# YongonY/NBLDPC

Measured on AMD Instinct MI355X. Metric: decoded codewords/sec @ 50 iters, GF(256) N=512 rate-1/2, higher is better.
Workload: dtype f64

## Files before the change

### nbldpc_amd/csrc/nbl_api.cpp

```cpp
#include <hip/hip_runtime.h>
#include <cstdio>
#include <cstdlib>
#include <cstring>
#include <chrono>
#include <cmath>
#include <string>
#include <thread>
#include <vector>
#include "../../include/nbldpc.h"
#include "nbl_kernels.h"
#include "nbl_osd.h"

static thread_local std::string g_create_error;

struct nbl_decoder {
	int device = -1;
	nbl_params prm{};
	nbl_params_ext ext{};
	bool osd_on = false;
	bool osd_acc = false;
	NblOsdDev osd{};
	double osd_factor = 0.0;
	double *osd_S = nullptr;
	NblGraphDev g{};
	NblWork w{};
	std::vector<void *> graph_allocs;
	int *d_e2c_map = nullptr;
	int cap = 0;
	size_t ws_bytes = 0;
	double *d_Lin = nullptr;
	uint8_t *d_conv8 = nullptr;
	hipStream_t stream = nullptr;
	bool record_state = false;
	bool all_dc4 = false;
	int min_dc = 0;
	bool all_dv2 = false;
	double *c2v_alt = nullptr;
	double *c2v_zero = nullptr;
	const double *last_c2v = nullptr;
	bool last_fused = false;
	int dm_order = 0, dm_L = 0;
	double *d_cons = nullptr;
	int *d_src = nullptr;
	double *d_rx = nullptr;
	size_t d_rx_cap = 0;
	std::vector<double> h_cons;
	uint32_t *d_jump = nullptr;
	uint32_t *d_state = nullptr;
	uint8_t *d_txi = nullptr;
	double *d_fn = nullptr;
	uint32_t *d_fidx = nullptr;
	double *d_farg = nullptr, *d_fval = nullptr;
	unsigned *d_fcount = nullptr;
	uint32_t *h_fidx = nullptr;
	double *h_farg = nullptr, *h_fval = nullptr;
	size_t noise_cap = 0, flag_cap = 0;
	double last_flag_frac = 0.0;
	hipStream_t stream2 = nullptr;
	double *d_rxs[2] = {nullptr, nullptr};
	size_t d_rxs_cap[2] = {0, 0};
	int rxs_B[2] = {0, 0};
	struct Tx {
		bool on = false;
		int crc_len = 0, random_msg = 0, K = 0, nb = 0, nw = 0, nwg = 0, mb = 0, period = 1, par_mod = 0;
		unsigned long long *T = nullptr, *G = nullptr;
		int *keep = nullptr;
		uint32_t *crc_col = nullptr;
		int16_t *phase_of = nullptr;
		uint8_t *seq = nullptr;
		uint16_t *pn = nullptr;
		unsigned long long *u = nullptr;
		uint8_t *bits = nullptr;
		size_t cap = 0;
		uint8_t *code[2] = {nullptr, nullptr}, *txi[2] = {nullptr, nullptr};
		size_t slot_cap[2] = {0, 0};
		int tx_B[2] = {0, 0};
		int *dec[2] = {nullptr, nullptr};
		size_t dec_cap[2] = {0, 0};
// ... 10 lines not shown
	int *d_active = nullptr;
	bool use_compact = true;
	bool use_graph = false;
	int force_generic = 0;
	bool profiling = false;
	hipEvent_t ev[2] = {nullptr, nullptr};
	int *h_ndone = nullptr;
	std::vector<hipEvent_t> pev;
	double ms[4] = {0, 0, 0, 0};
	long long launches[3] = {0, 0, 0};
	int last_B = 0;
	std::vector<int> h_coff, h_cvar, h_ch;
	std::vector<uint16_t> h_mul;
	std::string err;
};

#define HIP_TRY_E(errstr, call)                                                                    \
	do {                                                                                           \
		hipError_t e_ = (call);                                                                    \
		if (e_ != hipSuccess) {                                                                    \
			(errstr) = std::string(#call) + ": " + hipGetErrorString(e_);                          \
			return NBL_ERR_HIP;                                                                    \
		}                                                                                          \
	} while (0)
#define HIP_TRY(dec, call) HIP_TRY_E((dec)->err, call)

static int ilog2(int q)
{
	int p = 0;
	while ((1 << p) < q) p++;
	return p;
}

template <typename T> static nbl_status upload(nbl_decoder *d, const std::vector<T> &h, const T **dst)
{
	void *p = nullptr;
	HIP_TRY(d, hipMalloc(&p, h.size() * sizeof(T) + 16));
	d->graph_allocs.push_back(p);
	HIP_TRY(d, hipMemcpy(p, h.data(), h.size() * sizeof(T), hipMemcpyHostToDevice));
	*dst = (const T *)p;
	return NBL_OK;
}

static void drop_graphs(nbl_decoder *d)
{
	for (auto &ge : d->gexec)
		if (ge) (void)hipGraphExecDestroy(ge);
	d->gexec.clear();
}

static void free_workspace(nbl_decoder *d)
{
	drop_graphs(d);
	void *ptrs[] = {d->w.Lch, d->w.v2c, d->w.c2v, d->w.post, d->w.dec, d->w.out, d->w.iters, d->w.done, d->d_Lin, d->d_conv8, d->c2v_alt, d->w.edge_dec, d->d_active, d->c2v_zero, d->osd_S};
	d->osd_S = nullptr;
	d->c2v_zero = nullptr;
	d->d_active = nullptr;
	d->w.active = nullptr;
	d->c2v_alt = nullptr;
	for (void *p : ptrs)
		if (p) (void)hipFree(p);
	d->w.Lch = d->w.v2c = d->w.c2v = d->w.post = nullptr;
	d->w.dec = d->w.out = d->w.iters = d->w.edge_dec = nullptr;
	d->w.done = nullptr;
	d->d_Lin = nullptr;
	d->d_conv8 = nullptr;
	d->cap = 0;
	d->ws_bytes = 0;
}

static bool small_enabled()
{
	static const bool on = !getenv("NBL_NO_SMALL");
	return on;
}

static bool small_shape(const nbl_decoder *d)
{
	if (!small_enabled()) return false;
	const nbl_params &p = d->prm;
	if (p.method == NBL_METHOD_TEMS && d->all_dv2 && nbl_tems64_applicable(d->g, d->all_dc4, p.tems_nr, p.tems_nc)) return false;
	if (p.method == NBL_METHOD_BP && nbl_bp64_applicable(d->g, d->all_dc4)) return false;
	if (p.method == NBL_METHOD_EMS) return nbl_small_applicable(d->g, p.method, d->min_dc, p.ems_nm, p.ems_nc);
	if (p.method == NBL_METHOD_TEMS) return nbl_small_applicable(d->g, p.method, d->min_dc, 0, p.tems_nc);
	if (p.method == NBL_METHOD_BP) return nbl_small_applicable(d->g, p.method, d->min_dc, 0, 0);
	return false;
}

static bool ems64_shape(const nbl_decoder *d)
{
	return small_enabled() && d->prm.method == NBL_METHOD_EMS && nbl_ems64_applicable(d->g, d->min_dc, d->prm.ems_nm, d->prm.ems_nc);
}

static bool fused_shape(const nbl_decoder *d)
{
	if (small_shape(d) || ems64_shape(d)) return d->g.c_nbr != nullptr;
	if (!d->all_dv2) return false;
	if (d->prm.method == NBL_METHOD_EMS) return nbl_ems256_applicable(d->g, d->all_dc4, d->prm.ems_nm, d->prm.ems_nc);
	if (d->prm.method == NBL_METHOD_TEMS)
		return nbl_tems64_applicable(d->g, d->all_dc4, d->prm.tems_nr, d->prm.tems_nc) || nbl_tems256_applicable(d->g, d->all_dc4, d->prm.tems_nr, d->prm.tems_nc);
	if (d->prm.method == NBL_METHOD_BP) return nbl_bp256_applicable(d->g, d->all_dc4) || nbl_bp64_applicable(d->g, d->all_dc4);
	return false;
}

static nbl_status ensure_workspace(nbl_decoder *d, int B)
{
	const bool want_v2c = d->prm.method != NBL_METHOD_EMS || !fused_shape(d) || d->record_state || d->force_generic != 0;
	const bool want_post = d->record_state || d->osd_acc;
	if (B <= d->cap && (!want_post || d->w.post) && (!want_v2c || d->w.v2c)) return NBL_OK;
	int cap = B > d->cap ? B : d->cap;
	free_workspace(d);
	const size_t q = d->g.q, N = d->g.N, E = d->g.E;
	size_t bytes = 0;
	auto alloc = [&](void **p, size_t n) -> hipError_t { bytes += n; return hipMalloc(p, n); };
	HIP_TRY(d, alloc((void **)&d->w.Lch, (size_t)cap * N * q * 8));
	if (want_v2c) HIP_TRY(d, alloc((void **)&d->w.v2c, (size_t)cap * E * q * 8));
	HIP_TRY(d, alloc((void **)&d->w.c2v, (size_t)cap * E * q * 8));
	if (fused_shape(d)) {
		HIP_TRY(d, alloc((void **)&d->c2v_alt, (size_t)cap * E * q * 8));
		HIP_TRY(d, alloc((void **)&d->c2v_zero, E * q * 8));
		HIP_TRY(d, hipMemset(d->c2v_zero, 0, E * q * 8));
	}
	if (want_post) HIP_TRY(d, alloc((void **)&d->w.post, (size_t)cap * N * q * 8));
	if (d->osd_acc) HIP_TRY(d, alloc((void **)&d->osd_S, (size_t)cap * N * d->g.p * 8));
	HIP_TRY(d, alloc((void **)&d->w.dec, (size_t)cap * N * 4));
	if (d->prm.method != NBL_METHOD_EMS) HIP_TRY(d, alloc((void **)&d->w.edge_dec, (size_t)cap * E * 4));
	HIP_TRY(d, alloc((void **)&d->w.out, (size_t)cap * N * 4));
	HIP_TRY(d, alloc((void **)&d->w.iters, (size_t)cap * 4));
	HIP_TRY(d, alloc((void **)&d->w.done, (size_t)cap));
	HIP_TRY(d, alloc((void **)&d->d_active, (size_t)cap * 4));
	d->cap = cap;
	d->ws_bytes = bytes;
	return NBL_OK;
}

extern "C" int32_t nbl_abi_version(void) { return NBL_ABI_VERSION; }

extern "C" const char *nbl_last_error(const nbl_decoder *dec)
{
	if (!dec) return g_create_error.c_str();
	if (dec->err2.empty()) return dec->err.c_str();
	if (dec->err.empty()) return dec->err2.c_str();
	static thread_local std::string both;
	both = dec->err + " | channel: " + dec->err2;
	return both.c_str();
}

extern "C" size_t nbl_workspace_bytes(const nbl_decoder *dec) { return dec ? dec->ws_bytes : 0; }

static nbl_status fail_create(nbl_decoder *d, nbl_status st, const std::string &msg)
{
	g_create_error = msg.empty() && d ? d->err : msg;
	if (d) nbl_destroy(d);
	return st;
}

extern "C" nbl_status nbl_create(const nbl_code_desc *code, const uint16_t *gf_mul, const uint16_t *gf_inv,
                                 const nbl_params *params, int device, nbl_decoder **out)
{
	return nbl_create_ex(code, gf_mul, gf_inv, params, nullptr, device, out);
}

extern "C" nbl_status nbl_create_ex(const nbl_code_desc *code, const uint16_t *gf_mul, const uint16_t *gf_inv,
                                    const nbl_params *params, const nbl_params_ext *ext, int device, nbl_decoder **out)
{
	return nbl_create_osd(code, gf_mul, gf_inv, params, ext, nullptr, device, out);
}

static void g_gauss_eliminate(std::vector<std::vector<uint8_t>> &m, int col_length, int row_length, std::vector<int> &order)
{
	for (int row = 0; row < row_length; row++) {
		int col = order[row];
		if (m[row][col] == 0) {
			bool exchanged = false;
			for (int up = row + 1; up < row_length; up++)
				if (m[up][col] != 0) {
					for (int i = 0; i < col_length; i++) m[row][i] ^= m[up][i];
					exchanged = true;
					break;
				}
			if (!exchanged) {
				const int flag = row;
				row--;
// ... 280 lines not shown
	(void)hipDeviceSynchronize();
	free_workspace(d);
	for (void *p : d->graph_allocs) (void)hipFree(p);
	if (d->d_src) (void)hipFree(d->d_src);
	if (d->d_cons) (void)hipFree(d->d_cons);
	if (d->d_rx) (void)hipFree(d->d_rx);
	for (double *p : d->d_rxs)
		if (p) (void)hipFree(p);
	if (d->stream2) { (void)hipStreamSynchronize(d->stream2); (void)hipStreamDestroy(d->stream2); }
	for (void *p : {(void *)d->d_jump, (void *)d->d_state, (void *)d->d_txi, (void *)d->d_fn, (void *)d->d_fidx, (void *)d->d_farg, (void *)d->d_fval, (void *)d->d_fcount})
		if (p) (void)hipFree(p);
	for (void *p : {(void *)d->h_fidx, (void *)d->h_farg, (void *)d->h_fval})
		if (p) (void)hipHostFree(p);
	free_transmitter(d);
	for (auto &e : d->ev)
		if (e) (void)hipEventDestroy(e);
	if (d->h_ndone) (void)hipHostFree(d->h_ndone);
	for (auto &e : d->pev) (void)hipEventDestroy(e);
	if (d->stream) (void)hipStreamDestroy(d->stream);
	delete d;
}

extern "C" nbl_status nbl_set_profiling(nbl_decoder *d, int32_t on)
{
	if (!d) return NBL_ERR_ARG;
	d->profiling = on != 0;
	return NBL_OK;
}

extern "C" nbl_status nbl_debug_force_generic(nbl_decoder *d, int32_t on)
{
	if (!d) return NBL_ERR_ARG;
	d->force_generic = on;
	return NBL_OK;
}

extern "C" int32_t nbl_debug_graph_windows(nbl_decoder *d)
{
	int n = 0;
	if (d)
		for (auto &ge : d->gexec) n += ge != nullptr;
	return n;
}

extern "C" nbl_status nbl_debug_stamps(nbl_decoder *d, int32_t on, unsigned long long out[16])
{
	if (!d) return NBL_ERR_ARG;
	d->err.clear();
	HIP_TRY(d, hipSetDevice(d->device));
	if (out && d->w.stamps) {
		HIP_TRY(d, hipStreamSynchronize(d->stream));
		HIP_TRY(d, hipDeviceSynchronize());
		HIP_TRY(d, hipMemcpy(out, d->w.stamps, 16 * 8, hipMemcpyDeviceToHost));
	}
	if (on && !d->w.stamps) {
		void *p = nullptr;
		HIP_TRY(d, hipMalloc(&p, 16 * 8));
		d->graph_allocs.push_back(p);
		d->w.stamps = (unsigned long long *)p;
	}
	if (d->w.stamps && on) HIP_TRY(d, hipMemset(d->w.stamps, 0, 16 * 8));
	if (!on) d->w.stamps = nullptr;
	return NBL_OK;
}

extern "C" nbl_status nbl_set_record_state(nbl_decoder *d, int32_t on)
{
	if (!d) return NBL_ERR_ARG;
	d->record_state = on != 0;
	return NBL_OK;
}

extern "C" nbl_status nbl_last_timing(nbl_decoder *d, double ms[4], int64_t launches[3])
{
	if (!d) return NBL_ERR_ARG;
	if (ms) memcpy(ms, d->ms, sizeof d->ms);
	if (launches) for (int i = 0; i < 3; i++) launches[i] = d->launches[i];
	return NBL_OK;
}

static nbl_status launch_cn(nbl_decoder *d, const NblRun &r, hipStream_t st)
{
	const bool small_on = small_shape(d);
	switch (d->prm.method) {
	case NBL_METHOD_EMS:
		if (d->force_generic != 1 && nbl_ems256_applicable(d->g, d->all_dc4, r.nm, r.nc)) HIP_TRY(d, nbl_launch_cn_ems256(d->g, d->w, r, false, st));
		else if (d->force_generic != 1 && small_on) HIP_TRY(d, nbl_launch_cn_ems_small(d->g, d->w, r, false, st));
		else if (d->force_generic != 1 && ems64_shape(d)) HIP_TRY(d, nbl_launch_cn_ems64(d->g, d->w, r, false, st));
		else HIP_TRY(d, nbl_launch_cn_ems(d->g, d->w, r, st));
		break;
	case NBL_METHOD_TEMS:
		if (d->force_generic != 1 && nbl_tems64_applicable(d->g, d->all_dc4, r.nr, r.nc)) HIP_TRY(d, nbl_launch_cn_tems64(d->g, d->w, r, false, st));
		else if (d->force_generic != 1 && nbl_tems256_applicable(d->g, d->all_dc4, r.nr, r.nc)) HIP_TRY(d, nbl_launch_cn_tems256(d->g, d->w, r, false, st));
		else if (d->force_generic != 1 && small_on) HIP_TRY(d, nbl_launch_cn_tems_small(d->g, d->w, r, false, st));
		else HIP_TRY(d, nbl_launch_cn_tems(d->g, d->w, r, st));
		break;
	case NBL_METHOD_BP:
		if (d->force_generic != 1 && nbl_bp256_applicable(d->g, d->all_dc4)) HIP_TRY(d, nbl_launch_cn_bp256(d->g, d->w, r, false, st));
		else if (d->force_generic != 1 && nbl_bp64_applicable(d->g, d->all_dc4)) HIP_TRY(d, nbl_launch_cn_bp64(d->g, d->w, r, false, st));
		else if (d->force_generic != 1 && small_on) HIP_TRY(d, nbl_launch_cn_bp_small(d->g, d->w, r, false, st));
		else HIP_TRY(d, nbl_launch_cn_bp(d->g, d->w, r, st));
		break;
	case NBL_METHOD_BS_TEMS: HIP_TRY(d, nbl_launch_cn_bstems(d->g, d->w, r, st)); break;
	default: d->err = "check-node kernel for this method is not built yet"; return NBL_ERR_UNSUPPORTED;
	}
	return NBL_OK;
}

struct IterCtx {
	nbl_decoder *d;
	NblRun r;
	bool damp, fused;
	double *bufA, *bufB;
	const double *zeros = nullptr;
	int batch = 0;
// ... 880 lines not shown
```

### nbldpc_amd/csrc/nbl_cn_ems256.hip

```cpp
#include <hip/hip_runtime.h>
#ifndef NBL_EMS_PRUNE
#define NBL_EMS_PRUNE 1
#endif
#include <type_traits>
#include "nbl_device.h"
#include "nbl_kernels.h"

#ifndef NBL_WHATIF
#define NBL_WHATIF 0
#endif

namespace {

constexpr int Q = 256;

struct ListEnt { double v; int t8; int tt; };

#define WSYNC() __builtin_amdgcn_fence(__ATOMIC_ACQ_REL, "wavefront")

template <int CTRL, int ROW_MASK = 0xF>
__device__ __forceinline__ double dpp_mov_f64(double x)
{
	int lo = __builtin_amdgcn_update_dpp(__double2loint(x), __double2loint(x), CTRL, ROW_MASK, 0xF, false);
	int hi = __builtin_amdgcn_update_dpp(__double2hiint(x), __double2hiint(x), CTRL, ROW_MASK, 0xF, false);
	return __hiloint2double(hi, lo);
}

__device__ __forceinline__ double wave_max_f64(double x)
{
	x = dmax(x, dpp_mov_f64<0xB1>(x));
	x = dmax(x, dpp_mov_f64<0x4E>(x));
	x = dmax(x, dpp_mov_f64<0x141>(x));
	x = dmax(x, dpp_mov_f64<0x140>(x));
	x = dmax(x, dpp_mov_f64<0x142, 0xA>(x));
	x = dmax(x, dpp_mov_f64<0x143, 0xC>(x));
	return read_lane_f64(x, 63);
}

__device__ __forceinline__ int wave_scan_add(int x)
{
	x += __builtin_amdgcn_update_dpp(0, x, 0x111, 0xF, 0xF, false);
	x += __builtin_amdgcn_update_dpp(0, x, 0x112, 0xF, 0xF, false);
	x += __builtin_amdgcn_update_dpp(0, x, 0x114, 0xF, 0xF, false);
	x += __builtin_amdgcn_update_dpp(0, x, 0x118, 0xF, 0xF, false);
	x += __builtin_amdgcn_update_dpp(0, x, 0x142, 0xA, 0xF, false);
	x += __builtin_amdgcn_update_dpp(0, x, 0x143, 0xC, 0xF, false);
	return x;
}

__device__ __forceinline__ int wave_max_i32(int x)
{
	constexpr int ID = (int)0x80000000;
	auto mx = [](int a, int b) { return a > b ? a : b; };
	x = mx(x, __builtin_amdgcn_update_dpp(ID, x, 0xB1, 0xF, 0xF, false));
	x = mx(x, __builtin_amdgcn_update_dpp(ID, x, 0x4E, 0xF, 0xF, false));
// ... 122 lines not shown
		int best = -1;
#pragma unroll
		for (int i = 0; i < 4; i++) {
			const int a = __builtin_amdgcn_inverse_ballot_w64(eq[i]) ? mh.at_slot(i) : -1;
			best = a > best ? a : best;
		}
		const int amax = wave_max_i32(best);
#pragma unroll
		for (int i = 0; i < 4; i++) {
			const uint64_t hit = __ballot(__builtin_amdgcn_inverse_ballot_w64(eq[i]) && mh.at_slot(i) == amax);
			member[i] |= hit;
			eq[i] &= ~hit;
		}
	}
}

__device__ __forceinline__ void finish_members(SelState &s, int nm, uint64_t (&member)[4], int hinv, int poly, int lane)
{
	int cgt = 0, ceq = 0;
#pragma unroll
	for (int i = 0; i < 4; i++) { cgt += __popcll(s.gt[i]); ceq += __popcll(s.eq[i]); }
	const int need = nm - cgt;
#pragma unroll
	for (int i = 0; i < 4; i++) member[i] = s.gt[i];
	if (need == ceq) {
#pragma unroll
		for (int i = 0; i < 4; i++) member[i] |= s.eq[i];
	} else {
		finish_ties(member, s.eq, need, hinv, poly, lane);
	}
}

}

template <int NMT, bool FUSED, int NC>
__global__ __launch_bounds__(64) void cn_ems_q256_dc4_kernel(NblGraphDev g, NblWork w, NblRun r)
{
	constexpr int NM = NMT < 0 ? -NMT : NMT;
	constexpr bool VARNM = NMT < 0;
	const int nmr = VARNM ? r.nm : NM;
	constexpr int LOGNM = (NM == 8) ? 3 : (NM == 16) ? 4 : (NM == 32) ? 5 : 6;
#if NBL_WHATIF == 5
	__shared__ __attribute__((aligned(16))) char smem[13 * 1024];
#elif NBL_WHATIF == 6
	__shared__ __attribute__((aligned(16))) char smem[19 * 1024];
#else
	__shared__ __attribute__((aligned(16))) char smem[3 * Q * 8 + 4 * NM * 8 + 4 * NM * 8];
#endif
	const int lane = lane_id();
	const NblXcdSlot xs = nbl_xcd_slot(g.M);
	const int m = xs.unit, b = nbl_codeword(w, r, xs.slot);
	if (b < 0) return;
	if (!r.fixed_iters && w.done[b]) return;
#if NBL_EMS_PRUNE
	const bool tryf = NC >= 2 && r.fixed_iters && w.done[b];
#else
	const bool tryf = false;
#endif
	const int c0 = g.coff[m];

	double *const B0 = (double *)smem, *const B1 = B0 + Q, *const B2 = B1 + Q;
	double *const lstv = B2 + Q;
	int2 *const lstt = (int2 *)(lstv + 4 * NM);
	auto list_at = [&](int j, int k) {
		ListEnt e;
		e.v = lstv[j * NM + k];
		const int2 o = lstt[j * NM + k];
		e.t8 = o.x;
		e.tt = o.y;
		return e;
	};

#ifdef NBL_EMS_STAMPS
	unsigned long long st_t0 = 0, st_acc[15] = {0, 0, 0, 0, 0, 0, 0, 0, 0, 0, 0, 0, 0, 0, 0};
	const bool st_on = (w.stamps != nullptr) && ((blockIdx.x & 63) == 0);
#define STAMP(i) do { if (st_on) { unsigned long long t1_ = clock64(); st_acc[i] += t1_ - st_t0; st_t0 = t1_; } } while (0)
#define STAMP_COUNT(i) do { if (st_on) st_acc[i]++; } while (0)
	if (st_on) st_t0 = clock64();
#elif defined(NBL_EMS_MARKS)
#define STAMP(i) asm volatile("; NBLMARK " #i)
#define STAMP_COUNT(i) do { } while (0)
#else
#define STAMP(i) do { } while (0)
#define STAMP_COUNT(i) do { } while (0)
#endif

	const double *V = w.v2c + (size_t)b * g.E * Q;
	double *C = w.c2v + ((size_t)b * g.E + c0) * Q;

	uint2 toff[4];
#define TOFF(j, i) ((int)((((i) & 2) ? toff[j].y : toff[j].x) >> (16 * ((i) & 1))) & 0xffff)
#pragma unroll
	for (int j = 0; j < 4; j++) toff[j] = ((const uint2 *)g.ems_toff)[(size_t)(c0 + j) * 64 + lane];

	double v[4][4];
	if (!FUSED) {
#pragma unroll
		for (int j = 0; j < 4; j++) {
			const double2 *src = (const double2 *)(V + (size_t)g.c_epos[c0 + j] * Q);
			double2 d0 = src[lane], d1 = src[64 + lane];
			v[j][0] = (lane == 0) ? 0.0 : d0.x;
			v[j][1] = d0.y;
			v[j][2] = d1.x;
			v[j][3] = d1.y;
		}
	} else {
		const double *Cp = w.c2v_prev + (w.c2v_prev_shared ? (size_t)0 : (size_t)b * g.E * Q);
		double2 l0[4], l1[4], a0[4], a1[4], b0[4], b1[4];
		int nvar[4], eidx[4];
		bool ownA[4];
		const int *row = g.dv2_row + (size_t)m * 16;
#pragma unroll
		for (int j = 0; j < 4; j++) {
			const int n = row[j], cpA = row[4 + j], cpB = row[8 + j], e = row[12 + j] & 0x7fffffff;
#if NBL_WHATIF == 11
			const double2 *pl = (const double2 *)(w.Lch + ((size_t)(b & 7) * g.N + n) * Q);
#else
			const double2 *pl = (const double2 *)(w.Lch + ((size_t)b * g.N + n) * Q);
#endif
			const double2 *pa = (const double2 *)(Cp + (size_t)cpA * Q);
			const double2 *pb = (const double2 *)(Cp + (size_t)cpB * Q);
#if NBL_WHATIF == 4
			l0[j].x = (double)(long long)(pl + lane) * -1e-9; l0[j].y = l0[j].x * 1.5; l1[j].x = l0[j].x * 0.7; l1[j].y = l0[j].x * 0.3;
			a0[j].x = (double)(long long)(pa + lane) * -1e-9; a0[j].y = a0[j].x * 1.25; a1[j].x = a0[j].x * 0.6; a1[j].y = a0[j].x * 0.2;
			b0[j].x = (double)(long long)(pb + lane) * -1e-9; b0[j].y = b0[j].x * 1.125; b1[j].x = b0[j].x * 0.9; b1[j].y = b0[j].x * 0.4;
#else
			l0[j] = pl[lane]; l1[j] = pl[64 + lane];
			a0[j] = pa[lane]; a1[j] = pa[64 + lane];
			b0[j] = pb[lane]; b1[j] = pb[64 + lane];
#endif
			nvar[j] = n; eidx[j] = e;
			ownA[j] = row[12 + j] < 0;
		}
#pragma unroll
		for (int j = 0; j < 4; j++) {
			const int n = nvar[j], e = eidx[j];
			double post[4] = {(l0[j].x + a0[j].x) + b0[j].x, (l0[j].y + a0[j].y) + b0[j].y, (l1[j].x + a1[j].x) + b1[j].x,
			                  (l1[j].y + a1[j].y) + b1[j].y};
			if (ownA[j]) {
				v[j][0] = post[0] - a0[j].x; v[j][1] = post[1] - a0[j].y; v[j][2] = post[2] - a1[j].x; v[j][3] = post[3] - a1[j].y;
			} else {
				asm volatile("");
				v[j][0] = post[0] - b0[j].x; v[j][1] = post[1] - b0[j].y; v[j][2] = post[2] - b1[j].x; v[j][3] = post[3] - b1[j].y;
			}
			if (lane == 0) v[j][0] = 0.0;
			if (ownA[j]) {
				if (lane == 0) post[0] = 0.0;
				const double locp = dmax(dmax(post[0], post[1]), dmax(post[2], post[3]));
				const int kp = key32(locp);
				const double pm = wave_max_exact(locp, kp, wave_max_i32(kp));
				uint64_t hit[4];
#pragma unroll
				for (int i = 0; i < 4; i++) hit[i] = __ballot(post[i] == pm);
				const int arg = lowest_sym(hit);
				if (lane == 0) w.dec[(size_t)b * g.N + n] = (pm > 0.0) ? arg : 0;
				if (w.post) {
					double2 *pp = (double2 *)(w.post + ((size_t)b * g.N + n) * Q);
					double2 p01, p23;
					p01.x = post[0]; p01.y = post[1]; p23.x = post[2]; p23.y = post[3];
					pp[lane] = p01;
					pp[64 + lane] = p23;
				}
			}
			if (w.store_v2c) {
				double2 *pv = (double2 *)(w.v2c + ((size_t)b * g.E + e) * Q);
				double2 v01, v23;
				v01.x = v[j][0]; v01.y = v[j][1]; v23.x = v[j][2]; v23.y = v[j][3];
				pv[lane] = v01;
				pv[64 + lane] = v23;
			}
		}
	}
	STAMP(0);

	double mtop[4], lmin[4];
	double sec[4] = {0, 0, 0, 0};
	int ztop[4];
#pragma unroll
	for (int j = 0; j < 4; j++) {
		const double loc = dmax(dmax(v[j][0], v[j][1]), dmax(v[j][2], v[j][3]));
		const int k = key32(loc);
		mtop[j] = wave_max_exact(loc, k, wave_max_i32(k));
		constexpr int KEY_3E38 = 0x7f61b1e6;
		const int kmin = wave_min_i32(k);
		const double lf = (double)unkey32(kmin < KEY_3E38 ? kmin : KEY_3E38);
		lmin[j] = ((lf - (mtop[j] - lf) * 0x1p-20) - __builtin_fabs(lf) * 0x1p-22) - 0x1p-120;
		uint64_t eqm[4];
#pragma unroll
		for (int i = 0; i < 4; i++) eqm[i] = __ballot(v[j][i] == mtop[j]);
		const int topa = highest_sym(eqm);
		const int tl = (topa & 127) >> 1;
		const unsigned twl = (unsigned)__builtin_amdgcn_readlane((int)toff[j].x, tl), twh = (unsigned)__builtin_amdgcn_readlane((int)toff[j].y, tl);
		const unsigned tw = (topa & 128) ? twh : twl;
		ztop[j] = (int)((tw >> (16 * (topa & 1))) & 0xffffu) >> 3;
#if NBL_EMS_PRUNE
		if (tryf) {
			const int ts = (topa & 1) + 2 * (topa >> 7);
			const double mate = (ts == 0) ? v[j][1] : (ts == 1) ? v[j][0] : (ts == 2) ? v[j][3] : v[j][2];
			const double far = (ts & 2) ? dmax(v[j][0], v[j][1]) : dmax(v[j][2], v[j][3]);
			const double loc2 = (lane == tl) ? dmax(mate, far) : loc;
			const double sf = (double)unkey32(wave_max_i32(key32(loc2)));
			sec[j] = uniform_f64((sf + __builtin_fabs(sf) * 0x1p-22) + 0x1p-120);
		}
#endif
	}
	STAMP(1);

	double S[4][4];
#pragma unroll
	for (int x = 0; x < 4; x++)
#pragma unroll
		for (int i = 0; i < 4; i++) S[x][i] = -NBL_DBL_MAX;
	const int ztot = ztop[0] ^ ztop[1] ^ ztop[2] ^ ztop[3];
	const int lane16 = lane << 4;
#pragma unroll
	for (int j = 0; j < 4; j++) {
		char *const Uj = (char *)(j == 1 ? B1 : j == 2 ? B2 : B0);
		WSYNC();
#pragma unroll
		for (int i = 0; i < 4; i++) *(double *)(Uj + TOFF(j, i)) = v[j][i];
		WSYNC();
#pragma unroll
		for (int x = 0; x < 4; x++) {
			if (x == j) continue;
			const int shift = ztot ^ ztop[x] ^ ztop[j];
			const int ad = lane16 ^ ((shift & 0xFE) << 3);
			const double2 ra = *(const double2 *)(Uj + ad), rb = *(const double2 *)(Uj + (ad ^ 1024));
			auto upd = [&](double u0, double u1, double u2, double u3) {
				const double uu[4] = {u0, u1, u2, u3};
#pragma unroll
				for (int i = 0; i < 4; i++) {
					double acc = 0.0;
#pragma unroll
					for (int o = 0; o < 4; o++) {
						if (o == x) continue;
						acc = acc + ((o == j) ? uu[i] : mtop[o]);
					}
					S[x][i] = dmax(S[x][i], acc);
				}
			};
			if (shift & 1) upd(ra.y, ra.x, rb.y, rb.x);
			else upd(ra.x, ra.y, rb.x, rb.y);
		}
		if (NC >= 2) {
			const double2 d0 = *(const double2 *)(Uj + lane16), d1 = *(const double2 *)(Uj + lane16 + 1024);
			v[j][0] = d0.x; v[j][1] = d0.y; v[j][2] = d1.x; v[j][3] = d1.y;
		}
	}
	STAMP(5);

	int n0[4] = {0, 0, 0, 0}, nA[4] = {0, 0, 0, 0}, nC[4] = {0, 0, 0, 0};
	int cntl[4] = {nmr, nmr, nmr, nmr};
	bool fast = false;
	double thr[4] = {0, 0, 0, 0};
#if NBL_EMS_PRUNE
	if (tryf) {
		double flo[4];
#pragma unroll
		for (int x = 0; x < 4; x++) {
			const double lf = (double)unkey32(wave_min_i32(key32(dmin(dmin(S[x][0], S[x][1]), dmin(S[x][2], S[x][3])))));
			flo[x] = uniform_f64((lf - __builtin_fabs(lf) * 0x1p-22) - 0x1p-120);
		}
		auto pb = [&](int b, int c) { return dmax(mtop[b] + sec[c], sec[b] + mtop[c]); };
		const double p01 = pb(0, 1), p02 = pb(0, 2), p03 = pb(0, 3), p12 = pb(1, 2), p13 = pb(1, 3), p23 = pb(2, 3);
		auto low = [&](double f, double p) {
			const double t = f - p;
			return (t - (__builtin_fabs(f) + __builtin_fabs(p)) * 0x1p-40) - 0x1p-100;
		};
		thr[0] = uniform_f64(dmin(dmin(low(flo[1], p23), low(flo[2], p13)), low(flo[3], p12)));
		thr[1] = uniform_f64(dmin(dmin(low(flo[0], p23), low(flo[2], p03)), low(flo[3], p02)));
		thr[2] = uniform_f64(dmin(dmin(low(flo[0], p13), low(flo[1], p03)), low(flo[3], p01)));
		thr[3] = uniform_f64(dmin(dmin(low(flo[0], p12), low(flo[1], p02)), low(flo[2], p01)));
		fast = true;
#pragma unroll
		for (int j = 0; j < 4; j++) {
			int c = 0;
#pragma unroll
			for (int i = 0; i < 4; i++) c += __popcll(__ballot(!(v[j][i] < thr[j])));
			cntl[j] = c;
			fast = fast && c <= nmr;
		}
		if (!fast) cntl[0] = cntl[1] = cntl[2] = cntl[3] = nmr;
#ifdef NBL_EMS_STAMPS
		if (st_on) { st_acc[13] += fast ? 1 : 0; st_acc[14] += cntl[0] + cntl[1] + cntl[2] + cntl[3]; }
#endif
	}
#endif
	if (NC >= 2) {
		auto compact = [&](int j, const uint64_t (&member)[4]) {
			const int c0n = __popcll(member[0]), c2n = __popcll(member[2]), c1n = __popcll(member[1]);
			const int ne = c0n + c2n;
			n0[j] = ne;
			nA[j] = c0n;
			nC[j] = ne + c1n;
			const int base[4] = {j * NM, j * NM + ne, j * NM + c0n, j * NM + ne + c1n};
#pragma unroll
			for (int i = 0; i < 4; i++) {
				const int pos = __builtin_amdgcn_mbcnt_hi((uint32_t)(member[i] >> 32), __builtin_amdgcn_mbcnt_lo((uint32_t)member[i], base[i]));
				if (__builtin_amdgcn_inverse_ballot_w64(member[i])) {
					lstv[pos] = v[j][i];
					lstt[pos] = make_int2(sym_of(lane, i) << 3, (sym_of(lane, i) & 0x7E) << 3);
				}
			}
		};
		if (VARNM || fast) {
			WSYNC();
#pragma unroll
			for (int j = 0; j < 4; j++) {
				lstv[j * NM + (lane & (NM - 1))] = NBL_NEG_INF;
				lstt[j * NM + (lane & (NM - 1))] = make_int2((lane & (NM - 1)) << 3, 0);
			}
			WSYNC();
		}
		if (fast) {
#pragma unroll
			for (int j = 0; j < 4; j++) {
				uint64_t member[4];
#pragma unroll
				for (int i = 0; i < 4; i++) member[i] = __ballot(!(v[j][i] < thr[j]));
				compact(j, member);
			}
		} else {
			int bk[4][4];
			int *H = (int *)B0;
			int one;
			asm volatile("v_mov_b32 %0, 1" : "=v"(one));
			WSYNC();
			{
				int4 z4 = {0, 0, 0, 0};
#pragma unroll
				for (int i = 0; i < 4; i++) ((int4 *)H)[i * 64 + lane] = z4;
			}
			WSYNC();
#pragma unroll
			for (int j = 0; j < 4; j++) {
				const double scale = 256.0 * __builtin_amdgcn_rcp(mtop[j] - lmin[j]);
#pragma unroll
				for (int i = 0; i < 4; i++) {
					int bi;
// ... 327 lines not shown
```

### nbldpc_amd/csrc/nbl_common.h

```cpp
#pragma once
#include <stdint.h>

#define NBL_WAVE 64
#define NBL_MAXDC 8
#define NBL_MAXDV 8

struct NblGraphDev {
	int N, M, E, q, p, poly, maxdc, maxdv;
	const int *voff;
	const int *coff;
	const int *v_cpos;
	const int *c_epos;
	const int *c_var;
	const int *c_h;
	const int *c_hinv;
	const uint8_t *mul;
	const int *c_nbr;
	const unsigned long long *ems_toff;
	const int *dv2_row;
};

struct NblWork {
	double *Lch, *v2c, *c2v, *post;
	const double *c2v_prev;
	int c2v_prev_shared;
	int store_v2c;
	int *dec, *out, *iters;
	int *edge_dec;
	uint8_t *done;
	int *n_done;
	const int *active;
	const int *n_act;
	unsigned long long *stamps;
};

struct NblRun {
	int B;
	int iter, fixed_iters;
	int nm, nc, nr;
	double factor, offset;
	double damp_old, damp_new;
};
```

### nbldpc_amd/csrc/nbl_kernels.hip

```cpp
#include <hip/hip_runtime.h>
#include "nbl_device.h"
#include "nbl_kernels.h"

__global__ void init_kernel(const double *__restrict__ Lin, NblGraphDev g, NblWork w, int B, int write_v2c)
{
	const int q = g.q;
	long long total = (long long)B * g.N * q;
	for (long long i = (long long)blockIdx.x * blockDim.x + threadIdx.x; i < total; i += (long long)gridDim.x * blockDim.x) {
		int a = (int)(i % q);
		long long bn = i / q;
		if (Lin) w.Lch[i] = a ? Lin[bn * (q - 1) + (a - 1)] : 0.0;
	}
	long long etotal = (long long)B * g.E * q;
	if (!(write_v2c & 2))
		for (long long i = (long long)blockIdx.x * blockDim.x + threadIdx.x; i < etotal; i += (long long)gridDim.x * blockDim.x)
			w.c2v[i] = 0.0;
	if (write_v2c & 1) {
		for (long long i = (long long)blockIdx.x * blockDim.x + threadIdx.x; i < etotal; i += (long long)gridDim.x * blockDim.x) {
			int a = (int)(i % q);
			long long be = i / q;
			int e = (int)(be % g.E);
			long long b = be / g.E;
			int lo = 0, hi = g.N;
			while (hi - lo > 1) { int mid = (lo + hi) >> 1; if (g.voff[mid] <= e) lo = mid; else hi = mid; }
			w.v2c[i] = a ? (Lin ? Lin[(b * g.N + lo) * (q - 1) + (a - 1)] : w.Lch[(b * g.N + lo) * q + a]) : 0.0;
		}
	}
	for (long long i = (long long)blockIdx.x * blockDim.x + threadIdx.x; i < B; i += (long long)gridDim.x * blockDim.x) {
		w.done[i] = 0;
		w.iters[i] = 0;
	}
	if (blockIdx.x == 0 && threadIdx.x == 0) *w.n_done = 0;
}

__global__ __launch_bounds__(256) void demod_kernel(const double *__restrict__ rx, int L, double sigma_n, int mod_order, int p,
                                                    const double *__restrict__ cons, const int *__restrict__ src, NblGraphDev g,
                                                    NblWork w, int B)
{
	const int lane = lane_id();
	const long long node = (long long)blockIdx.x * (blockDim.x >> 6) + (threadIdx.x >> 6);
	if (node >= (long long)B * g.N) return;
	const int b = (int)(node / g.N), n = (int)(node % g.N), q = g.q;
	double *dst = w.Lch + ((size_t)b * g.N + n) * q;
	const double *r = rx + (size_t)b * L * 2;
	if (mod_order == 2) {
		double bl[8];
		for (int k = 0; k < 8; k++) {
			const int sidx = (k < p) ? src[n * p + k] : -1;
			bl[k] = (sidx < 0) ? 0.0 : -2 * r[2 * sidx] / (sigma_n * sigma_n);
		}
		for (int a = lane; a < q; a += 64) {
			double acc = 0;
#pragma unroll
			for (int k = 0; k < 8; k++)
				if (k < p && (a & (1 << k)) != 0) acc += bl[k];
			dst[a] = a ? acc : 0.0;
		}
	} else {
		const int sidx = src[n];
		const double c0r = cons[0], c0i = cons[1];
		const double re = sidx < 0 ? 0.0 : r[2 * sidx], im = sidx < 0 ? 0.0 : r[2 * sidx + 1];
		for (int a = lane; a < q; a += 64) {
			const double cr = cons[2 * a], ci = cons[2 * a + 1];
			const double num = (2 * re - c0r - cr) * (cr - c0r) + (2 * im - c0i - ci) * (ci - c0i);
			dst[a] = (a == 0 || sidx < 0) ? 0.0 : num / (2 * sigma_n * sigma_n);
		}
	}
}

template <int Q, bool DAMP>
__global__ __launch_bounds__(256) void vn_kernel(NblGraphDev g, NblWork w, NblRun r)
{
	constexpr int NS = Fld<Q>::NS;
	const int lane = lane_id();
	const long long node = (long long)blockIdx.x * (blockDim.x >> 6) + (threadIdx.x >> 6);
	if (node >= (long long)r.B * g.N) return;
	const int b = nbl_codeword(w, r, (int)(node / g.N)), n = (int)(node % g.N);
	if (b < 0) return;
	if (!r.fixed_iters && w.done[b]) return;

	const int e0 = g.voff[n], dv = g.voff[n + 1] - e0;
	const double *L = w.Lch + ((size_t)b * g.N + n) * Q;
	const double *C = w.c2v + (size_t)b * g.E * Q;
	double *V = w.v2c + ((size_t)b * g.E + e0) * Q;
// ... 576 lines not shown
```

Before: 116,100.

## Add per-check backoff hint gating the EMS fast-path attempt

```diff
diff --git a/nbldpc_amd/csrc/nbl_api.cpp b/nbldpc_amd/csrc/nbl_api.cpp
--- a/nbldpc_amd/csrc/nbl_api.cpp
+++ b/nbldpc_amd/csrc/nbl_api.cpp
@@ -24,6 +24,7 @@
 	double *osd_S = nullptr;
 	NblGraphDev g{};
 	NblWork w{};
+	unsigned long long gate_counts[512] = {};
 	std::vector<void *> graph_allocs;
 	int *d_e2c_map = nullptr;
 	int cap = 0;
@@ -140,7 +141,7 @@
 static void free_workspace(nbl_decoder *d)
 {
 	drop_graphs(d);
-	void *ptrs[] = {d->w.Lch, d->w.v2c, d->w.c2v, d->w.post, d->w.dec, d->w.out, d->w.iters, d->w.done, d->d_Lin, d->d_conv8, d->c2v_alt, d->w.edge_dec, d->d_active, d->c2v_zero, d->osd_S};
+	void *ptrs[] = {d->w.Lch, d->w.v2c, d->w.c2v, d->w.post, d->w.dec, d->w.out, d->w.iters, d->w.done, d->d_Lin, d->d_conv8, d->c2v_alt, d->w.edge_dec, d->d_active, d->c2v_zero, d->osd_S, d->w.ems_hint};
 	d->osd_S = nullptr;
 	d->c2v_zero = nullptr;
 	d->d_active = nullptr;
@@ -151,6 +152,7 @@
 	d->w.Lch = d->w.v2c = d->w.c2v = d->w.post = nullptr;
 	d->w.dec = d->w.out = d->w.iters = d->w.edge_dec = nullptr;
 	d->w.done = nullptr;
+	d->w.ems_hint = nullptr;
 	d->d_Lin = nullptr;
 	d->d_conv8 = nullptr;
 	d->cap = 0;
@@ -217,6 +219,8 @@
 	HIP_TRY(d, alloc((void **)&d->w.iters, (size_t)cap * 4));
 	HIP_TRY(d, alloc((void **)&d->w.done, (size_t)cap));
 	HIP_TRY(d, alloc((void **)&d->d_active, (size_t)cap * 4));
+	if (d->prm.method == NBL_METHOD_EMS && nbl_ems256_applicable(d->g, d->all_dc4, d->prm.ems_nm, d->prm.ems_nc))
+		HIP_TRY(d, alloc((void **)&d->w.ems_hint, (size_t)cap * d->g.M));
 	d->cap = cap;
 	d->ws_bytes = bytes;
 	return NBL_OK;
@@ -603,15 +607,31 @@
 		HIP_TRY(d, hipStreamSynchronize(d->stream));
 		HIP_TRY(d, hipDeviceSynchronize());
 		HIP_TRY(d, hipMemcpy(out, d->w.stamps, 16 * 8, hipMemcpyDeviceToHost));
+		HIP_TRY(d, hipMemcpy(d->gate_counts, d->w.stamps + 16, sizeof d->gate_counts, hipMemcpyDeviceToHost));
 	}
 	if (on && !d->w.stamps) {
 		void *p = nullptr;
-		HIP_TRY(d, hipMalloc(&p, 16 * 8));
+		HIP_TRY(d, hipMalloc(&p, (16 + 512) * 8));
 		d->graph_allocs.push_back(p);
 		d->w.stamps = (unsigned long long *)p;
 	}
-	if (d->w.stamps && on) HIP_TRY(d, hipMemset(d->w.stamps, 0, 16 * 8));
+	if (d->w.stamps && on) HIP_TRY(d, hipMemset(d->w.stamps, 0, (16 + 512) * 8));
 	if (!on) d->w.stamps = nullptr;
+	return NBL_OK;
+}
+
+extern "C" nbl_status nbl_debug_gate_counts(nbl_decoder *d, unsigned long long out[512])
+{
+	if (!d || !out) return NBL_ERR_ARG;
+	memcpy(out, d->gate_counts, sizeof d->gate_counts);
+	return NBL_OK;
+}
+
+extern "C" nbl_status nbl_debug_ems_try_all(nbl_decoder *d, int32_t on)
+{
+	if (!d) return NBL_ERR_ARG;
+	if ((d->w.ems_try != 0) != (on != 0)) drop_graphs(d);
+	d->w.ems_try = on ? 1 : 0;
 	return NBL_OK;
 }
 
diff --git a/nbldpc_amd/csrc/nbl_cn_ems256.hip b/nbldpc_amd/csrc/nbl_cn_ems256.hip
--- a/nbldpc_amd/csrc/nbl_cn_ems256.hip
+++ b/nbldpc_amd/csrc/nbl_cn_ems256.hip
@@ -1,6 +1,12 @@
 #include <hip/hip_runtime.h>
 #ifndef NBL_EMS_PRUNE
 #define NBL_EMS_PRUNE 1
+#endif
+#ifndef NBL_EMS_GATE_ZTOT
+#define NBL_EMS_GATE_ZTOT 0
+#endif
+#ifndef NBL_EMS_BACKOFF
+#define NBL_EMS_BACKOFF 3
 #endif
 #include <type_traits>
 #include "nbl_device.h"
@@ -230,9 +236,9 @@
 	if (b < 0) return;
 	if (!r.fixed_iters && w.done[b]) return;
 #if NBL_EMS_PRUNE
-	const bool tryf = NC >= 2 && r.fixed_iters && w.done[b];
-#else
-	const bool tryf = false;
+	const int cw_done = __builtin_amdgcn_readfirstlane((int)w.done[b]);
+	uint8_t *const hintp = (NC >= 2 && w.ems_hint) ? w.ems_hint + ((size_t)b * g.M + m) : nullptr;
+	const int hint = hintp ? __builtin_amdgcn_readfirstlane((int)*hintp) : 0;
 #endif
 	const int c0 = g.coff[m];
 
@@ -351,7 +357,6 @@
 	STAMP(0);
 
 	double mtop[4], lmin[4];
-	double sec[4] = {0, 0, 0, 0};
 	int ztop[4];
 #pragma unroll
 	for (int j = 0; j < 4; j++) {
@@ -370,16 +375,6 @@
 		const unsigned twl = (unsigned)__builtin_amdgcn_readlane((int)toff[j].x, tl), twh = (unsigned)__builtin_amdgcn_readlane((int)toff[j].y, tl);
 		const unsigned tw = (topa & 128) ? twh : twl;
 		ztop[j] = (int)((tw >> (16 * (topa & 1))) & 0xffffu) >> 3;
-#if NBL_EMS_PRUNE
-		if (tryf) {
-			const int ts = (topa & 1) + 2 * (topa >> 7);
-			const double mate = (ts == 0) ? v[j][1] : (ts == 1) ? v[j][0] : (ts == 2) ? v[j][3] : v[j][2];
-			const double far = (ts & 2) ? dmax(v[j][0], v[j][1]) : dmax(v[j][2], v[j][3]);
-			const double loc2 = (lane == tl) ? dmax(mate, far) : loc;
-			const double sf = (double)unkey32(wave_max_i32(key32(loc2)));
-			sec[j] = uniform_f64((sf + __builtin_fabs(sf) * 0x1p-22) + 0x1p-120);
-		}
-#endif
 	}
 	STAMP(1);
 
@@ -389,6 +384,13 @@
 #pragma unroll
 		for (int i = 0; i < 4; i++) S[x][i] = -NBL_DBL_MAX;
 	const int ztot = ztop[0] ^ ztop[1] ^ ztop[2] ^ ztop[3];
+#if NBL_EMS_PRUNE
+	const bool cand = NC >= 2 && (cw_done || (NBL_EMS_GATE_ZTOT && ztot == 0));
+	const bool tryf = NC >= 2 && (w.ems_try || (cand && hint == 0));
+	int hint_new = (cand && hint > 0) ? hint - 1 : hint;
+#else
+	const bool tryf = false;
+#endif
 	const int lane16 = lane << 4;
 #pragma unroll
 	for (int j = 0; j < 4; j++) {
@@ -437,6 +439,17 @@
 		for (int x = 0; x < 4; x++) {
 			const double lf = (double)unkey32(wave_min_i32(key32(dmin(dmin(S[x][0], S[x][1]), dmin(S[x][2], S[x][3])))));
 			flo[x] = uniform_f64((lf - __builtin_fabs(lf) * 0x1p-22) - 0x1p-120);
+		}
+		double sec[4];
+#pragma unroll
+		for (int j = 0; j < 4; j++) {
+			const int tl = (ztop[j] & 127) >> 1, ts = (ztop[j] & 1) + 2 * (ztop[j] >> 7);
+			const double mate = (ts == 0) ? v[j][1] : (ts == 1) ? v[j][0] : (ts == 2) ? v[j][3] : v[j][2];
+			const double far = (ts & 2) ? dmax(v[j][0], v[j][1]) : dmax(v[j][2], v[j][3]);
+			const double loc = dmax(dmax(v[j][0], v[j][1]), dmax(v[j][2], v[j][3]));
+			const double loc2 = (lane == tl) ? dmax(mate, far) : loc;
+			const double sf = (double)unkey32(wave_max_i32(key32(loc2)));
+			sec[j] = uniform_f64((sf + __builtin_fabs(sf) * 0x1p-22) + 0x1p-120);
 		}
 		auto pb = [&](int b, int c) { return dmax(mtop[b] + sec[c], sec[b] + mtop[c]); };
 		const double p01 = pb(0, 1), p02 = pb(0, 2), p03 = pb(0, 3), p12 = pb(1, 2), p13 = pb(1, 3), p23 = pb(2, 3);
@@ -448,20 +461,25 @@
 		thr[1] = uniform_f64(dmin(dmin(low(flo[0], p23), low(flo[2], p03)), low(flo[3], p02)));
 		thr[2] = uniform_f64(dmin(dmin(low(flo[0], p13), low(flo[1], p03)), low(flo[3], p01)));
 		thr[3] = uniform_f64(dmin(dmin(low(flo[0], p12), low(flo[1], p02)), low(flo[2], p01)));
-		fast = true;
+		fast = nmr < 64 ? (thr[0] > lmin[0] && thr[1] > lmin[1] && thr[2] > lmin[2] && thr[3] > lmin[3]) : true;
 #pragma unroll
 		for (int j = 0; j < 4; j++) {
-			int c = 0;
-#pragma unroll
-			for (int i = 0; i < 4; i++) c += __popcll(__ballot(!(v[j][i] < thr[j])));
-			cntl[j] = c;
-			fast = fast && c <= nmr;
+			if (fast) {
+				int c = 0;
+#pragma unroll
+				for (int i = 0; i < 4; i++) c += __popcll(__ballot(!(v[j][i] < thr[j])));
+				cntl[j] = c;
+				fast = c <= nmr;
+			}
 		}
 		if (!fast) cntl[0] = cntl[1] = cntl[2] = cntl[3] = nmr;
+		hint_new = fast ? 0 : NBL_EMS_BACKOFF;
 #ifdef NBL_EMS_STAMPS
 		if (st_on) { st_acc[13] += fast ? 1 : 0; st_acc[14] += cntl[0] + cntl[1] + cntl[2] + cntl[3]; }
-#endif
-	}
+		if (st_on && lane == 0) atomicAdd(&w.stamps[16 + (r.iter & 63) * 8 + (cw_done ? 4 : 0) + (ztot == 0 ? 2 : 0) + (fast ? 1 : 0)], 1ull);
+#endif
+	}
+	if (hintp && hint_new != hint && lane == 0) *hintp = (uint8_t)hint_new;
 #endif
 	if (NC >= 2) {
 		auto compact = [&](int j, const uint64_t (&member)[4]) {
diff --git a/nbldpc_amd/csrc/nbl_common.h b/nbldpc_amd/csrc/nbl_common.h
--- a/nbldpc_amd/csrc/nbl_common.h
+++ b/nbldpc_amd/csrc/nbl_common.h
@@ -32,6 +32,8 @@
 	const int *active;
 	const int *n_act;
 	unsigned long long *stamps;
+	uint8_t *ems_hint;
+	int ems_try;
 };
 
 struct NblRun {
diff --git a/nbldpc_amd/csrc/nbl_kernels.hip b/nbldpc_amd/csrc/nbl_kernels.hip
--- a/nbldpc_amd/csrc/nbl_kernels.hip
+++ b/nbldpc_amd/csrc/nbl_kernels.hip
@@ -30,6 +30,9 @@
 		w.done[i] = 0;
 		w.iters[i] = 0;
 	}
+	if (w.ems_hint)
+		for (long long i = (long long)blockIdx.x * blockDim.x + threadIdx.x; i < (long long)B * g.M; i += (long long)gridDim.x * blockDim.x)
+			w.ems_hint[i] = 0;
 	if (blockIdx.x == 0 && threadIdx.x == 0) *w.n_done = 0;
 }
 
```

Result: slower. 113,600 (-2.1%).

## Interleave per-edge ranking and LDS staging with the input loads in EMS check-node kernel

Applied to the files above, without the earlier changes.

```diff
diff --git a/nbldpc_amd/csrc/nbl_cn_ems256.hip b/nbldpc_amd/csrc/nbl_cn_ems256.hip
--- a/nbldpc_amd/csrc/nbl_cn_ems256.hip
+++ b/nbldpc_amd/csrc/nbl_cn_ems256.hip
@@ -229,12 +229,7 @@
 	const int m = xs.unit, b = nbl_codeword(w, r, xs.slot);
 	if (b < 0) return;
 	if (!r.fixed_iters && w.done[b]) return;
-#if NBL_EMS_PRUNE
-	const bool tryf = NC >= 2 && r.fixed_iters && w.done[b];
-#else
-	const bool tryf = false;
-#endif
-	const int c0 = g.coff[m];
+	const int c0 = 4 * m;
 
 	double *const B0 = (double *)smem, *const B1 = B0 + Q, *const B2 = B1 + Q;
 	double *const lstv = B2 + Q;
@@ -269,92 +264,23 @@
 #define TOFF(j, i) ((int)((((i) & 2) ? toff[j].y : toff[j].x) >> (16 * ((i) & 1))) & 0xffff)
 #pragma unroll
 	for (int j = 0; j < 4; j++) toff[j] = ((const uint2 *)g.ems_toff)[(size_t)(c0 + j) * 64 + lane];
+	int dn = 0;
+	if (NC >= 2 && NBL_EMS_PRUNE && r.fixed_iters) dn = w.done[b];
 
 	double v[4][4];
-	if (!FUSED) {
-#pragma unroll
-		for (int j = 0; j < 4; j++) {
-			const double2 *src = (const double2 *)(V + (size_t)g.c_epos[c0 + j] * Q);
-			double2 d0 = src[lane], d1 = src[64 + lane];
-			v[j][0] = (lane == 0) ? 0.0 : d0.x;
-			v[j][1] = d0.y;
-			v[j][2] = d1.x;
-			v[j][3] = d1.y;
-		}
-	} else {
-		const double *Cp = w.c2v_prev + (w.c2v_prev_shared ? (size_t)0 : (size_t)b * g.E * Q);
-		double2 l0[4], l1[4], a0[4], a1[4], b0[4], b1[4];
-		int nvar[4], eidx[4];
-		bool ownA[4];
-		const int *row = g.dv2_row + (size_t)m * 16;
-#pragma unroll
-		for (int j = 0; j < 4; j++) {
-			const int n = row[j], cpA = row[4 + j], cpB = row[8 + j], e = row[12 + j] & 0x7fffffff;
-#if NBL_WHATIF == 11
-			const double2 *pl = (const double2 *)(w.Lch + ((size_t)(b & 7) * g.N + n) * Q);
-#else
-			const double2 *pl = (const double2 *)(w.Lch + ((size_t)b * g.N + n) * Q);
-#endif
-			const double2 *pa = (const double2 *)(Cp + (size_t)cpA * Q);
-			const double2 *pb = (const double2 *)(Cp + (size_t)cpB * Q);
-#if NBL_WHATIF == 4
-			l0[j].x = (double)(long long)(pl + lane) * -1e-9; l0[j].y = l0[j].x * 1.5; l1[j].x = l0[j].x * 0.7; l1[j].y = l0[j].x * 0.3;
-			a0[j].x = (double)(long long)(pa + lane) * -1e-9; a0[j].y = a0[j].x * 1.25; a1[j].x = a0[j].x * 0.6; a1[j].y = a0[j].x * 0.2;
-			b0[j].x = (double)(long long)(pb + lane) * -1e-9; b0[j].y = b0[j].x * 1.125; b1[j].x = b0[j].x * 0.9; b1[j].y = b0[j].x * 0.4;
-#else
-			l0[j] = pl[lane]; l1[j] = pl[64 + lane];
-			a0[j] = pa[lane]; a1[j] = pa[64 + lane];
-			b0[j] = pb[lane]; b1[j] = pb[64 + lane];
-#endif
-			nvar[j] = n; eidx[j] = e;
-			ownA[j] = row[12 + j] < 0;
-		}
-#pragma unroll
-		for (int j = 0; j < 4; j++) {
-			const int n = nvar[j], e = eidx[j];
-			double post[4] = {(l0[j].x + a0[j].x) + b0[j].x, (l0[j].y + a0[j].y) + b0[j].y, (l1[j].x + a1[j].x) + b1[j].x,
-			                  (l1[j].y + a1[j].y) + b1[j].y};
-			if (ownA[j]) {
-				v[j][0] = post[0] - a0[j].x; v[j][1] = post[1] - a0[j].y; v[j][2] = post[2] - a1[j].x; v[j][3] = post[3] - a1[j].y;
-			} else {
-				asm volatile("");
-				v[j][0] = post[0] - b0[j].x; v[j][1] = post[1] - b0[j].y; v[j][2] = post[2] - b1[j].x; v[j][3] = post[3] - b1[j].y;
-			}
-			if (lane == 0) v[j][0] = 0.0;
-			if (ownA[j]) {
-				if (lane == 0) post[0] = 0.0;
-				const double locp = dmax(dmax(post[0], post[1]), dmax(post[2], post[3]));
-				const int kp = key32(locp);
-				const double pm = wave_max_exact(locp, kp, wave_max_i32(kp));
-				uint64_t hit[4];
-#pragma unroll
-				for (int i = 0; i < 4; i++) hit[i] = __ballot(post[i] == pm);
-				const int arg = lowest_sym(hit);
-				if (lane == 0) w.dec[(size_t)b * g.N + n] = (pm > 0.0) ? arg : 0;
-				if (w.post) {
-					double2 *pp = (double2 *)(w.post + ((size_t)b * g.N + n) * Q);
-					double2 p01, p23;
-					p01.x = post[0]; p01.y = post[1]; p23.x = post[2]; p23.y = post[3];
-					pp[lane] = p01;
-					pp[64 + lane] = p23;
-				}
-			}
-			if (w.store_v2c) {
-				double2 *pv = (double2 *)(w.v2c + ((size_t)b * g.E + e) * Q);
-				double2 v01, v23;
-				v01.x = v[j][0]; v01.y = v[j][1]; v23.x = v[j][2]; v23.y = v[j][3];
-				pv[lane] = v01;
-				pv[64 + lane] = v23;
-			}
-		}
-	}
-	STAMP(0);
-
 	double mtop[4], lmin[4];
 	double sec[4] = {0, 0, 0, 0};
 	int ztop[4];
-#pragma unroll
-	for (int j = 0; j < 4; j++) {
+	const int lane16 = lane << 4;
+	constexpr bool EARLY3 = 4 * NM * 16 >= Q * 8;
+	auto stage_buf = [&](int j) { return (char *)(j == 1 ? B1 : j == 2 ? B2 : (j == 3 && EARLY3) ? lstv : B0); };
+#if NBL_EMS_PRUNE
+	bool tryf = false;
+#else
+	const bool tryf = false;
+#endif
+
+	auto rank0 = [&](int j) __attribute__((always_inline)) {
 		const double loc = dmax(dmax(v[j][0], v[j][1]), dmax(v[j][2], v[j][3]));
 		const int k = key32(loc);
 		mtop[j] = wave_max_exact(loc, k, wave_max_i32(k));
@@ -380,8 +306,115 @@
 			sec[j] = uniform_f64((sf + __builtin_fabs(sf) * 0x1p-22) + 0x1p-120);
 		}
 #endif
-	}
-	STAMP(1);
+	};
+	auto stage = [&](int j) __attribute__((always_inline)) {
+		char *const Uj = stage_buf(j);
+		WSYNC();
+#pragma unroll
+		for (int i = 0; i < 4; i++) *(double *)(Uj + TOFF(j, i)) = v[j][i];
+		WSYNC();
+		if (NC >= 2) {
+			const double2 d0 = *(const double2 *)(Uj + lane16), d1 = *(const double2 *)(Uj + lane16 + 1024);
+			v[j][0] = d0.x; v[j][1] = d0.y; v[j][2] = d1.x; v[j][3] = d1.y;
+		}
+	};
+
+	if (!FUSED) {
+#pragma unroll
+		for (int j = 0; j < 4; j++) {
+			const double2 *src = (const double2 *)(V + (size_t)g.c_epos[c0 + j] * Q);
+			double2 d0 = src[lane], d1 = src[64 + lane];
+			v[j][0] = (lane == 0) ? 0.0 : d0.x;
+			v[j][1] = d0.y;
+			v[j][2] = d1.x;
+			v[j][3] = d1.y;
+		}
+#if NBL_EMS_PRUNE
+		tryf = __builtin_amdgcn_readfirstlane(dn) != 0;
+#endif
+		STAMP(0);
+#pragma unroll
+		for (int j = 0; j < 4; j++) {
+			rank0(j);
+			STAMP(1);
+			if (j < 3 || EARLY3) stage(j);
+			STAMP(5);
+		}
+	} else {
+		const double *Cp = w.c2v_prev + (w.c2v_prev_shared ? (size_t)0 : (size_t)b * g.E * Q);
+		double2 l0[4], l1[4], a0[4], a1[4], b0[4], b1[4];
+		int nvar[4], eidx[4];
+		bool ownA[4];
+		const int *row = g.dv2_row + (size_t)m * 16;
+#pragma unroll
+		for (int j = 0; j < 4; j++) {
+			const int n = row[j], cpA = row[4 + j], cpB = row[8 + j], e = row[12 + j] & 0x7fffffff;
+#if NBL_WHATIF == 11
+			const double2 *pl = (const double2 *)(w.Lch + ((size_t)(b & 7) * g.N + n) * Q);
+#else
+			const double2 *pl = (const double2 *)(w.Lch + ((size_t)b * g.N + n) * Q);
+#endif
+			const double2 *pa = (const double2 *)(Cp + (size_t)cpA * Q);
+			const double2 *pb = (const double2 *)(Cp + (size_t)cpB * Q);
+#if NBL_WHATIF == 4
+			l0[j].x = (double)(long long)(pl + lane) * -1e-9; l0[j].y = l0[j].x * 1.5; l1[j].x = l0[j].x * 0.7; l1[j].y = l0[j].x * 0.3;
+			a0[j].x = (double)(long long)(pa + lane) * -1e-9; a0[j].y = a0[j].x * 1.25; a1[j].x = a0[j].x * 0.6; a1[j].y = a0[j].x * 0.2;
+			b0[j].x = (double)(long long)(pb + lane) * -1e-9; b0[j].y = b0[j].x * 1.125; b1[j].x = b0[j].x * 0.9; b1[j].y = b0[j].x * 0.4;
+#else
+			l0[j] = pl[lane]; l1[j] = pl[64 + lane];
+			a0[j] = pa[lane]; a1[j] = pa[64 + lane];
+			b0[j] = pb[lane]; b1[j] = pb[64 + lane];
+#endif
+			nvar[j] = n; eidx[j] = e;
+			ownA[j] = row[12 + j] < 0;
+		}
+#pragma unroll
+		for (int j = 0; j < 4; j++) {
+			const int n = nvar[j], e = eidx[j];
+			double post[4] = {(l0[j].x + a0[j].x) + b0[j].x, (l0[j].y + a0[j].y) + b0[j].y, (l1[j].x + a1[j].x) + b1[j].x,
+			                  (l1[j].y + a1[j].y) + b1[j].y};
+			if (ownA[j]) {
+				v[j][0] = post[0] - a0[j].x; v[j][1] = post[1] - a0[j].y; v[j][2] = post[2] - a1[j].x; v[j][3] = post[3] - a1[j].y;
+			} else {
+				asm volatile("");
+				v[j][0] = post[0] - b0[j].x; v[j][1] = post[1] - b0[j].y; v[j][2] = post[2] - b1[j].x; v[j][3] = post[3] - b1[j].y;
+			}
+			if (lane == 0) v[j][0] = 0.0;
+			if (ownA[j]) {
+				if (lane == 0) post[0] = 0.0;
+				const double locp = dmax(dmax(post[0], post[1]), dmax(post[2], post[3]));
+				const int kp = key32(locp);
+				const double pm = wave_max_exact(locp, kp, wave_max_i32(kp));
+				uint64_t hit[4];
+#pragma unroll
+				for (int i = 0; i < 4; i++) hit[i] = __ballot(post[i] == pm);
+				const int arg = lowest_sym(hit);
+				if (lane == 0) w.dec[(size_t)b * g.N + n] = (pm > 0.0) ? arg : 0;
+				if (w.post) {
+					double2 *pp = (double2 *)(w.post + ((size_t)b * g.N + n) * Q);
+					double2 p01, p23;
+					p01.x = post[0]; p01.y = post[1]; p23.x = post[2]; p23.y = post[3];
+					pp[lane] = p01;
+					pp[64 + lane] = p23;
+				}
+			}
+			if (w.store_v2c) {
+				double2 *pv = (double2 *)(w.v2c + ((size_t)b * g.E + e) * Q);
+				double2 v01, v23;
+				v01.x = v[j][0]; v01.y = v[j][1]; v23.x = v[j][2]; v23.y = v[j][3];
+				pv[lane] = v01;
+				pv[64 + lane] = v23;
+			}
+#if NBL_EMS_PRUNE
+			if (j == 0) tryf = __builtin_amdgcn_readfirstlane(dn) != 0;
+#endif
+			STAMP(0);
+			rank0(j);
+			STAMP(1);
+			if (j < 3 || EARLY3) stage(j);
+			STAMP(5);
+		}
+	}
 
 	double S[4][4];
 #pragma unroll
@@ -389,14 +422,10 @@
 #pragma unroll
 		for (int i = 0; i < 4; i++) S[x][i] = -NBL_DBL_MAX;
 	const int ztot = ztop[0] ^ ztop[1] ^ ztop[2] ^ ztop[3];
-	const int lane16 = lane << 4;
 #pragma unroll
 	for (int j = 0; j < 4; j++) {
-		char *const Uj = (char *)(j == 1 ? B1 : j == 2 ? B2 : B0);
-		WSYNC();
-#pragma unroll
-		for (int i = 0; i < 4; i++) *(double *)(Uj + TOFF(j, i)) = v[j][i];
-		WSYNC();
+		if (j == 3 && !EARLY3) stage(j);
+		const char *const Uj = stage_buf(j);
 #pragma unroll
 		for (int x = 0; x < 4; x++) {
 			if (x == j) continue;
@@ -419,11 +448,8 @@
 			if (shift & 1) upd(ra.y, ra.x, rb.y, rb.x);
 			else upd(ra.x, ra.y, rb.x, rb.y);
 		}
-		if (NC >= 2) {
-			const double2 d0 = *(const double2 *)(Uj + lane16), d1 = *(const double2 *)(Uj + lane16 + 1024);
-			v[j][0] = d0.x; v[j][1] = d0.y; v[j][2] = d1.x; v[j][3] = d1.y;
-		}
-	}
+	}
+	WSYNC();
 	STAMP(5);
 
 	int n0[4] = {0, 0, 0, 0}, nA[4] = {0, 0, 0, 0}, nC[4] = {0, 0, 0, 0};
```

New measurement: 113,900 before, 114,400 after (median of 6 runs). About the same (+0.5%).
